# carry4985/ORB_SLAM2_MAP

Measured on AMD Instinct MI355X. Metric: frames/sec ORB extract+match (640x480, 1000 feat), higher is better.
Workload: dtype u8; 1 GPU; C2: synthetic 640x480 RGB-D stream, 1000 features, 8 levels, extract + BF-Hamming match of consecutive frames; resident_frame_pool=1024, sequences=1, parallelism=1 sequence per GPU, schedule_name=best, extraction_parts=1

## Files before the change

### orb_slam2_map_amd/csrc/extractor.hip

```cpp
#include "common.h"

#include <atomic>
#include <chrono>
#include <thread>
#include <tuple>
#include <type_traits>
#include <utility>
#include "trig_base.h"
#include "pyramid_view.h"

#include <algorithm>
#include <cfloat>
#include <cmath>
#include <cstdlib>
#include <cstring>
#include <vector>

namespace orbgpu {

constexpr int EDGE = 19;
constexpr int BORDER0 = EDGE - 3;
constexpr int HALF_PATCH = 15;
constexpr int PATCH = 31;
constexpr float CELL_W = 30.f;
// ... 59 lines not shown

struct Src0 {
    const uint8_t *p;
    size_t frame_stride;
    uint32_t pitch;
    int direct;
};
constexpr int BLUR0_OX = EDGE + 1;

__device__ __forceinline__ uint32_t rowoff(int row, int pitch) { return __umul24((unsigned)row, (unsigned)pitch); }

constexpr int PYR_ROWS = 8;

__global__ __launch_bounds__(256) void k_border0(const uint8_t *__restrict__ src, size_t stride,
                                                 size_t frame_stride, uint8_t *__restrict__ pyr,
                                                 size_t frame_pyr, const LevelGeom *__restrict__ geom)
{
    const LevelGeom g = geom[0];
    const int ndw = g.pitch >> 2;
    int bx, f;
    xcd_frame_block(bx, f);
    const int item = bx * 256 + threadIdx.x;
    const int rg = item / ndw;
    const int x4 = (item - rg * ndw) * 4;
    if (rg * PYR_ROWS >= g.h + 2 * EDGE)
        return;
    const int sx0 = x4 - EDGE;
    const bool interior = sx0 >= 0 && sx0 + 7 < g.w;
#pragma unroll 4
    for (int rr = 0; rr < PYR_ROWS; rr++) {
        const int py = rg * PYR_ROWS + rr;
        if (py >= g.h + 2 * EDGE)
            break;
        const int sy = reflect101(py - EDGE, g.h);
        const uint8_t *s = src + (size_t)f * frame_stride + __umul24((unsigned)sy, (unsigned)stride);
        uint32_t v = 0;
        if (interior && ((reinterpret_cast<uintptr_t>(s) & 3) == 0)) {
            const uint32_t *s32 = reinterpret_cast<const uint32_t *>(s) + (sx0 >> 2);
            v = __builtin_amdgcn_alignbyte(s32[1], s32[0], sx0 & 3);
        } else {
#pragma unroll
            for (int k = 0; k < 4; k++) {
                int px = min(x4 + k, g.w + 2 * EDGE - 1);
                int sx = reflect101(px - EDGE, g.w);
                v |= (uint32_t)s[sx] << (8 * k);
            }
        }
        *reinterpret_cast<uint32_t *>(pyr + (size_t)f * frame_pyr + g.plane_off + rowoff(py, g.pitch) + x4) = v;
    }
}

constexpr int BORDER_ROWS = 4;

struct BorderCol {
    uint32_t d;
    uint32_t sel;
};

__global__ __launch_bounds__(256) void k_border0_fast(const uint8_t *__restrict__ src, size_t stride, size_t frame_stride,
                                                      uint8_t *__restrict__ pyr, size_t frame_pyr,
                                                      const LevelGeom *__restrict__ geom,
                                                      const BorderCol *__restrict__ cols)
{
    const LevelGeom g = geom[0];
    const int n16 = g.pitch >> 4;
    int bx, f;
    xcd_frame_block(bx, f);
    const int item = bx * 256 + threadIdx.x;
    const int rg = item / n16;
    const int c16 = item - rg * n16;
    if (rg * BORDER_ROWS >= g.h + 2 * EDGE)
        return;
    const uint4 t01 = reinterpret_cast<const uint4 *>(cols)[c16 * 2], t23 = reinterpret_cast<const uint4 *>(cols)[c16 * 2 + 1];
    const uint8_t *sf = src + (size_t)f * frame_stride;
    uint8_t *dst = pyr + (size_t)f * frame_pyr + g.plane_off + c16 * 16;
    const bool interior = c16 >= 2 && c16 * 16 - EDGE + 15 < g.w - 1 && c16 * 4 - 5 + 4 < (g.w >> 2);
    struct __attribute__((packed, aligned(4))) Win {
        uint32_t d[5];
    };
    if (interior) {
        Win wn[BORDER_ROWS];
#pragma unroll
        for (int rr = 0; rr < BORDER_ROWS; rr++) {
            const int py = min(rg * BORDER_ROWS + rr, g.h + 2 * EDGE - 1);
            wn[rr] = *reinterpret_cast<const Win *>(sf + __umul24((unsigned)reflect101(py - EDGE, g.h), (unsigned)stride) +
                                                    (c16 * 16 - 20));
        }
#pragma unroll
        for (int rr = 0; rr < BORDER_ROWS; rr++) {
            const int py = rg * BORDER_ROWS + rr;
            if (py >= g.h + 2 * EDGE)
                break;
            uint4 v;
            v.x = __builtin_amdgcn_alignbyte(wn[rr].d[1], wn[rr].d[0], 1);
            v.y = __builtin_amdgcn_alignbyte(wn[rr].d[2], wn[rr].d[1], 1);
            v.z = __builtin_amdgcn_alignbyte(wn[rr].d[3], wn[rr].d[2], 1);
            v.w = __builtin_amdgcn_alignbyte(wn[rr].d[4], wn[rr].d[3], 1);
            *reinterpret_cast<uint4 *>(dst + rowoff(py, g.pitch)) = v;
        }
        return;
    }
#pragma unroll
    for (int rr = 0; rr < BORDER_ROWS; rr++) {
        const int py = rg * BORDER_ROWS + rr;
        if (py >= g.h + 2 * EDGE)
            break;
        const uint32_t *s32 = reinterpret_cast<const uint32_t *>(sf + __umul24((unsigned)reflect101(py - EDGE, g.h), (unsigned)stride));
        uint4 v;
        v.x = __builtin_amdgcn_perm(s32[t01.x + 1], s32[t01.x], t01.y);
        v.y = __builtin_amdgcn_perm(s32[t01.z + 1], s32[t01.z], t01.w);
        v.z = __builtin_amdgcn_perm(s32[t23.x + 1], s32[t23.x], t23.y);
        v.w = __builtin_amdgcn_perm(s32[t23.z + 1], s32[t23.z], t23.w);
        *reinterpret_cast<uint4 *>(dst + rowoff(py, g.pitch)) = v;
    }
}

__global__ __launch_bounds__(256) void k_resize_level(uint8_t *__restrict__ pyr, size_t frame_pyr,
                                                      const LevelGeom *__restrict__ geom, int level,
                                                      const XTab *__restrict__ xtab,
                                                      const YTab *__restrict__ ytab)
{
    const LevelGeom g = geom[level];
    const LevelGeom gs = geom[level - 1];
    const int x4 = (blockIdx.x * 256 + threadIdx.x) * 4;
    const int py = blockIdx.y;
    const int f = blockIdx.z;
    if (x4 >= g.pitch)
        return;
    const int dy = reflect101(py - EDGE, g.h);
    const YTab yt = ytab[g.ytab_off + dy];
    const uint8_t *base = pyr + (size_t)f * frame_pyr + gs.plane_off + rowoff(EDGE, gs.pitch) + EDGE;
    const uint8_t *S0 = base + rowoff(yt.sy0, gs.pitch);
    const uint8_t *S1 = base + rowoff(yt.sy1, gs.pitch);
    uint32_t v = 0;
#pragma unroll
    for (int k = 0; k < 4; k++) {
        int px = min(x4 + k, g.w + 2 * EDGE - 1);
        int dx = reflect101(px - EDGE, g.w);
        const XTab xt = xtab[g.xtab_off + dx];
        int t0 = S0[xt.sx] * xt.a0 + S0[xt.sx1] * xt.a1;
        int t1 = S1[xt.sx] * xt.a0 + S1[xt.sx1] * xt.a1;
        int o = ((((int)yt.b0 * (t0 >> 4)) >> 16) + (((int)yt.b1 * (t1 >> 4)) >> 16) + 2) >> 2;
        v |= (uint32_t)(o & 0xFF) << (8 * k);
    }
    *reinterpret_cast<uint32_t *>(pyr + (size_t)f * frame_pyr + g.plane_off + rowoff(py, g.pitch) + x4) = v;
}

struct ResizeStrip {
    uint32_t base_q;
};

typedef unsigned short us2 __attribute__((ext_vector_type(2)));

template <bool REUSE, bool DIRECT>
__global__ __launch_bounds__(256) void k_resize_fast(uint8_t *__restrict__ pyr, size_t frame_pyr,
                                                     const LevelGeom *__restrict__ geom, int level,
                                                     const ResizeStrip *__restrict__ strips,
                                                     const uint4 *__restrict__ sels, const uint4 *__restrict__ wts,
                                                     const YRow *__restrict__ yrows, int strip_off, int rows, Src0 s0)
{
    const LevelGeom g = geom[level];
    const LevelGeom gs = geom[level - 1];
    const int ndw = g.pitch >> 2;
    int bx, f;
    xcd_frame_block(bx, f);
    const int item = bx * 256 + threadIdx.x;
    const int rg = item / ndw;
    const int sdw = item - rg * ndw;
    if (rg * rows >= g.h + 2 * EDGE)
        return;
    const uint32_t bq = strips[strip_off + sdw].base_q;
    const uint32_t sh = (bq >> 16) & 3u;
    const uint4 sel = sels[strip_off + sdw], wt = wts[strip_off + sdw];
    const uint32_t selv[4] = {sel.x, sel.y, sel.z, sel.w}, wv[4] = {wt.x, wt.y, wt.z, wt.w};
    uint8_t *fb = pyr + (size_t)f * frame_pyr;
    const uint8_t *sb = DIRECT ? s0.p + (size_t)f * s0.frame_stride : fb;
    const int spitch = DIRECT ? (int)s0.pitch : gs.pitch;
    const uint32_t base = (DIRECT ? 0u : (uint32_t)gs.plane_off + (uint32_t)EDGE * (uint32_t)gs.pitch) + (bq & 0xFFFFu);
    const bool edge = DIRECT && ((bq >> 18) & 1u) != 0u;
    const uint32_t dst = (uint32_t)g.plane_off + (uint32_t)sdw * 4u;
    YRow yts[PYR_ROWS];
#pragma unroll
    for (int rr = 0; rr < PYR_ROWS; rr++)
        yts[rr] = yrows[g.yrow_off + min(rg * rows + rr, g.h + 2 * EDGE - 1)];
    int kept_row = -1, kept[4] = {0, 0, 0, 0};
#pragma unroll
    for (int rr = 0; rr < PYR_ROWS; rr++) {
        const int py = rg * rows + rr;
        if (rr >= rows || py >= g.h + 2 * EDGE)
            break;
        const YRow yt = yts[rr];
        const uint32_t *S1 = reinterpret_cast<const uint32_t *>(sb + (base + rowoff(yt.sy1, spitch)));
        uint32_t c0 = S1[0], c1 = S1[1];
        const uint32_t c2 = S1[2];
        if (DIRECT) {
            c0 = edge ? c1 : c0;
            c1 = edge ? c2 : c1;
        }
        int t0[4];
        if (!REUSE || yt.sy0 != kept_row) {
            const uint32_t *S0 = reinterpret_cast<const uint32_t *>(sb + (base + rowoff(yt.sy0, spitch)));
            uint32_t a0 = S0[0], a1 = S0[1];
            const uint32_t a2 = S0[2];
            if (DIRECT) {
                a0 = edge ? a1 : a0;
                a1 = edge ? a2 : a1;
            }
            const uint32_t lo = __builtin_amdgcn_alignbyte(a1, a0, sh), hi = __builtin_amdgcn_alignbyte(a2, a1, sh);
#pragma unroll
            for (int k = 0; k < 4; k++) {
                const uint32_t p0 = __builtin_amdgcn_perm(hi, lo, selv[k]);
                t0[k] = (int)__builtin_amdgcn_udot2(__builtin_bit_cast(us2, p0), __builtin_bit_cast(us2, wv[k]), 0u, false);
            }
        } else {
#pragma unroll
            for (int k = 0; k < 4; k++)
                t0[k] = kept[k];
        }
        uint32_t v = 0;
        const uint32_t lo1 = __builtin_amdgcn_alignbyte(c1, c0, sh), hi1 = __builtin_amdgcn_alignbyte(c2, c1, sh);
#pragma unroll
        for (int k = 0; k < 4; k++) {
            const uint32_t p1 = __builtin_amdgcn_perm(hi1, lo1, selv[k]);
            const int t1 = (int)__builtin_amdgcn_udot2(__builtin_bit_cast(us2, p1), __builtin_bit_cast(us2, wv[k]), 0u, false);
            const int o = ((__mul24(yt.b0, t0[k] >> 4) >> 16) + (__mul24(yt.b1, t1 >> 4) >> 16) + 2) >> 2;
            v |= (uint32_t)o << (8 * k);
            kept[k] = t1;
        }
        kept_row = yt.sy1;
        *reinterpret_cast<uint32_t *>(fb + (dst + rowoff(py, g.pitch))) = v;
    }
}

constexpr int MAX_CELL = 66;

typedef short pk16 __attribute__((ext_vector_type(2)));
__device__ __forceinline__ pk16 as_pk(uint32_t u) { return __builtin_bit_cast(pk16, u); }
__device__ __forceinline__ uint32_t as_u32(pk16 v) { return __builtin_bit_cast(uint32_t, v); }
__device__ __forceinline__ pk16 pkmin(pk16 a, pk16 b) { return __builtin_elementwise_min(a, b); }
__device__ __forceinline__ pk16 pkmax(pk16 a, pk16 b) { return __builtin_elementwise_max(a, b); }

typedef _Float16 pkh __attribute__((ext_vector_type(2)));
__device__ __forceinline__ pkh as_h(pk16 v) { return __builtin_bit_cast(pkh, v); }
__device__ __forceinline__ pk16 h_as_pk(pkh v) { return __builtin_bit_cast(pk16, v); }
__device__ __forceinline__ pkh hmax3(pkh a, pkh b, pkh c)
{
    return __builtin_elementwise_maximum(__builtin_elementwise_maximum(a, b), c);
}
__device__ __forceinline__ pkh hmin3(pkh a, pkh b, pkh c)
{
    return __builtin_elementwise_minimum(__builtin_elementwise_minimum(a, b), c);
}

__device__ __forceinline__ pk16 fast_score_pk(pk16 c, const pk16 p[16])
{
    pkh v[16], m2[8], m4[8], t[8];
#pragma unroll
    for (int k = 0; k < 16; k++)
        v[k] = as_h(p[k]);
#pragma unroll
    for (int i = 0; i < 8; i++)
        m2[i] = __builtin_elementwise_maximum(v[2 * i + 1], v[(2 * i + 2) & 15]);
#pragma unroll
    for (int i = 0; i < 8; i++)
        m4[i] = __builtin_elementwise_maximum(m2[i], m2[(i + 1) & 7]);
#pragma unroll
    for (int i = 0; i < 8; i++)
        t[i] = hmax3(m4[i], m4[(i + 2) & 7], __builtin_elementwise_minimum(v[2 * i], v[(2 * i + 9) & 15]));
    const pkh A = __builtin_elementwise_minimum(hmin3(hmin3(t[0], t[1], t[2]), hmin3(t[3], t[4], t[5]), t[6]), t[7]);
#pragma unroll
    for (int i = 0; i < 8; i++)
        m2[i] = __builtin_elementwise_minimum(v[2 * i + 1], v[(2 * i + 2) & 15]);
#pragma unroll
    for (int i = 0; i < 8; i++)
        m4[i] = __builtin_elementwise_minimum(m2[i], m2[(i + 1) & 7]);
#pragma unroll
    for (int i = 0; i < 8; i++)
        t[i] = hmin3(m4[i], m4[(i + 2) & 7], __builtin_elementwise_maximum(v[2 * i], v[(2 * i + 9) & 15]));
    const pkh B = __builtin_elementwise_maximum(hmax3(hmax3(t[0], t[1], t[2]), hmax3(t[3], t[4], t[5]), t[6]), t[7]);
    typedef unsigned short pku16 __attribute__((ext_vector_type(2)));
    const pku16 cu = __builtin_bit_cast(pku16, c);
    const pku16 dk = __builtin_elementwise_sub_sat(cu, __builtin_bit_cast(pku16, A));
    const pku16 br = __builtin_elementwise_sub_sat(__builtin_bit_cast(pku16, B), cu);
    return __builtin_bit_cast(pk16, __builtin_elementwise_max(dk, br));
}

#define ORBGPU_SEL_EVEN(o) ((uint32_t)(o) | 0x0c00u | ((uint32_t)((o) + 2) << 16) | 0x0c000000u)
#define ORBGPU_SEL_ODD(o) ((uint32_t)((o) + 1) | 0x0c00u | ((uint32_t)((o) + 3) << 16) | 0x0c000000u)

struct Row3 {
    uint32_t d[3];
};

struct RowU {
    uint32_t f[8];
};
__device__ __forceinline__ void unpack_row(const Row3 &R, RowU &U)
{
#pragma unroll
    for (int o = 1; o <= 8; o++) {
        const int q = o >> 2;
        U.f[o - 1] = __builtin_amdgcn_perm(R.d[q < 2 ? q + 1 : 2], R.d[q], ORBGPU_SEL_EVEN(o & 3));
    }
}
template <int DX, int ODD> __device__ __forceinline__ pk16 ring_half(const RowU &R)
{
    return as_pk(R.f[4 + DX + ODD - 1]);
}

template <int ODD>
__device__ __forceinline__ pk16 fast_score_half(const RowU &r0, const RowU &r1, const RowU &r2, const RowU &r3,
                                                const RowU &r4, const RowU &r5, const RowU &r6)
{
    pk16 p[16];
    const pk16 c = ring_half<0, ODD>(r3);
    p[0] = ring_half<0, ODD>(r6);
    p[1] = ring_half<1, ODD>(r6);
    p[2] = ring_half<2, ODD>(r5);
    p[3] = ring_half<3, ODD>(r4);
    p[4] = ring_half<3, ODD>(r3);
    p[5] = ring_half<3, ODD>(r2);
    p[6] = ring_half<2, ODD>(r1);
    p[7] = ring_half<1, ODD>(r0);
    p[8] = ring_half<0, ODD>(r0);
    p[9] = ring_half<-1, ODD>(r0);
    p[10] = ring_half<-2, ODD>(r1);
    p[11] = ring_half<-3, ODD>(r2);
    p[12] = ring_half<-3, ODD>(r3);
    p[13] = ring_half<-3, ODD>(r4);
    p[14] = ring_half<-2, ODD>(r5);
    p[15] = ring_half<-1, ODD>(r6);
    return fast_score_pk(c, p);
}

template <int ODD>
__device__ __forceinline__ uint32_t fast_maybe_half(const RowU &r0, const RowU &r3, const RowU &r6, pkh tpk)
{
    const pkh c = as_h(ring_half<0, ODD>(r3));
    const pkh p0 = as_h(ring_half<0, ODD>(r6)), p4 = as_h(ring_half<3, ODD>(r3));
    const pkh p8 = as_h(ring_half<0, ODD>(r0)), p12 = as_h(ring_half<-3, ODD>(r3));
    const pkh bm = hmax3(__builtin_elementwise_minimum(p0, p4), __builtin_elementwise_minimum(p4, p8),
                         __builtin_elementwise_maximum(__builtin_elementwise_minimum(p8, p12), __builtin_elementwise_minimum(p12, p0)));
    const pkh dm = hmin3(__builtin_elementwise_maximum(p0, p4), __builtin_elementwise_maximum(p4, p8),
                         __builtin_elementwise_minimum(__builtin_elementwise_maximum(p8, p12), __builtin_elementwise_maximum(p12, p0)));
    const pk16 ci = h_as_pk(c), ti = h_as_pk(tpk);
    const uint32_t eb = as_u32((ci + ti) - h_as_pk(bm));
    const uint32_t ed = as_u32(h_as_pk(dm) - (ci - ti));
    return (eb | ed) & 0x80008000u;
}

struct StripGeom {
    int first[ORBGPU_MAX_LEVELS + 1];
    int nsx[ORBGPU_MAX_LEVELS];
    int nlevels;
};


constexpr int FD_OWN = 62;
constexpr int FD_QCAP = 512;
constexpr int FD_CELLS = 32;
constexpr int FD_EARLY_HOLD = 3;

struct DetectGeom {
    int first[ORBGPU_MAX_LEVELS + 1];
    int nsx[ORBGPU_MAX_LEVELS];
    int ncols[ORBGPU_MAX_LEVELS];
    int ctab_off[ORBGPU_MAX_LEVELS];
    int xfirst[ORBGPU_MAX_LEVELS];
    int nlevels;
};

struct ColumnInfo {
    uint32_t cellj;
    uint32_t flags;
};

struct DetectLane {
    int xrel, yrel;
    int cell_base;
    uint32_t cellj;
};

// ... 1953 lines not shown
    hipGraph_t graph = nullptr;
    hipGraphNode_t last = nullptr;
    hipError_t err = hipSuccess;

    Launcher() = default;
    explicit Launcher(hipStream_t s) : st(s) {}

    template <typename... P, typename... A> void launch(void (*kern)(P...), dim3 grid, dim3 block, size_t lds, A &&...a)
    {
        static_assert(sizeof...(P) == sizeof...(A), "kernel argument count");
        if (!graph) {
            hipLaunchKernelGGL(kern, grid, block, lds, st, static_cast<P>(a)...);
            return;
        }
        std::tuple<std::remove_cv_t<P>...> vals(static_cast<P>(a)...);
        void *ptrs[sizeof...(P) + 1];
        fill(ptrs, vals, std::index_sequence_for<P...>{});
        hipKernelNodeParams kp = {};
        kp.func = reinterpret_cast<void *>(kern);
        kp.gridDim = grid;
        kp.blockDim = block;
        kp.sharedMemBytes = (unsigned)lds;
        kp.kernelParams = ptrs;
        kp.extra = nullptr;
        add([&](hipGraphNode_t *n, const hipGraphNode_t *dep, size_t ndep) { return hipGraphAddKernelNode(n, graph, dep, ndep, &kp); });
    }
    int memset32(void *dst, size_t bytes)
    {
        if (!graph) {
            ORBGPU_HIP_TRY(hipMemsetAsync(dst, 0, bytes, st));
            return ORBGPU_OK;
        }
        hipMemsetParams mp = {};
        mp.dst = dst;
        mp.elementSize = 4;
        mp.width = bytes / 4;
        mp.height = 1;
        mp.pitch = bytes;
        mp.value = 0;
        add([&](hipGraphNode_t *n, const hipGraphNode_t *dep, size_t ndep) { return hipGraphAddMemsetNode(n, graph, dep, ndep, &mp); });
        return ORBGPU_OK;
    }

private:
    template <typename T, size_t... I> static void fill(void **ptrs, T &vals, std::index_sequence<I...>)
    {
        ((ptrs[I] = const_cast<void *>(static_cast<const void *>(&std::get<I>(vals)))), ...);
    }
    template <typename F> void add(F f)
    {
        hipGraphNode_t n = nullptr;
        const hipError_t e = f(&n, last ? &last : nullptr, last ? 1 : 0);
        if (e != hipSuccess && err == hipSuccess)
            err = e;
        if (e == hipSuccess)
            last = n;
    }
};

static int materialize_level0(orbgpu_extractor *e, const Src0 &s0, int batch, Launcher &L)
{
    const LevelGeom &g = e->geom[0];
    const LevelGeom *dg = e->d_geom.as<LevelGeom>();
    uint8_t *pyr = e->d_pyr.as<uint8_t>();
    const size_t stride = s0.pitch;
    if (e->border_fast && stride % 4 == 0 && s0.frame_stride % 4 == 0 && (reinterpret_cast<uintptr_t>(s0.p) & 3) == 0) {
        dim3 gridf(((g.pitch / 16) * ((g.h + 2 * EDGE + BORDER_ROWS - 1) / BORDER_ROWS) + 255) / 256, batch);
        L.launch(k_border0_fast, gridf, dim3(256), 0, s0.p, stride, s0.frame_stride, pyr, e->frame_pyr, dg,
                           e->d_bcol.as<BorderCol>());
    } else {
        dim3 grid(((g.pitch / 4) * ((g.h + 2 * EDGE + PYR_ROWS - 1) / PYR_ROWS) + 255) / 256, batch);
        L.launch(k_border0, grid, dim3(256), 0, s0.p, stride, s0.frame_stride, pyr, e->frame_pyr, dg);
    }
    if (!L.graph)
        ORBGPU_HIP_TRY(hipGetLastError());
    return ORBGPU_OK;
}

static void launch_blur(orbgpu_extractor *e, const Src0 &s0, int batch, Launcher &L, int which = 0)
{
    const int nl = e->nlevels;
    const LevelGeom *dg = e->d_geom.as<LevelGeom>();
    uint8_t *pyr = e->d_pyr.as<uint8_t>(), *blur = e->d_blur.as<uint8_t>();
    int strip0 = 0;
    if (s0.direct) {
        const LevelGeom &g = e->geom[0];
        const int nstrips = (g.w / 8) * ((g.h + BLUR_ROWS - 1) / BLUR_ROWS);
        if (which != 2)
            L.launch(k_blur0_direct, dim3((nstrips + 255) / 256, batch), dim3(256), 0, s0, blur, e->frame_pyr, dg);
        strip0 = e->blur_geom.first[1];
    }
    if (which == 1)
        return;
    if (e->blur_geom.first[nl] > strip0)
        L.launch(k_blur, dim3((e->blur_geom.first[nl] - strip0 + 255) / 256, batch), dim3(256), 0, pyr, blur,
                           e->frame_pyr, dg, e->blur_geom, strip0);
}

static int launch_pipeline(orbgpu_extractor *e, const uint8_t *d_gray, int batch, int w, int h, size_t stride,
                           size_t frame_stride, orbgpu_keypoint *d_kps, uint8_t *d_desc, int cap, int *d_n_out,
                           Launcher &L)
{
    hipStream_t st = L.st;
    const int nl = e->nlevels;
    const LevelGeom *dg = e->d_geom.as<LevelGeom>();
    uint8_t *pyr = e->d_pyr.as<uint8_t>();
    uint8_t *blur = e->d_blur.as<uint8_t>();
    int rc = e->d_aux.reserve(sizeof(KpAux) * (size_t)cap * batch);
    if (rc != ORBGPU_OK)
        return rc;
    const bool rec = L.graph != nullptr;
    const bool prof = !rec && e->profiling && e->prof_calls < orbgpu_extractor::PROF_SLOTS;
    if (prof && e->ev.empty()) {
        e->ev.resize((size_t)orbgpu_extractor::PROF_SLOTS * 2 * ST_COUNT, nullptr);
        for (auto &x : e->ev)
            ORBGPU_HIP_TRY(hipEventCreate(&x));
    }
    hipEvent_t *evs = prof ? &e->ev[(size_t)e->prof_calls * 2 * ST_COUNT] : nullptr;
#define BEGIN(stage, s) if (prof && (stage) == 0) ORBGPU_HIP_TRY(hipEventRecord(evs[0], s))
#define END(stage, s)                                                          \
    {                                                                          \
        if (prof)                                                              \
            ORBGPU_HIP_TRY(hipEventRecord(evs[1 + (stage)], s));               \
        if (!rec && e->stage_signal[stage])                                    \
            ORBGPU_HIP_TRY(hipEventRecord(e->stage_signal[stage], s));         \
        if (!rec && e->pipe_signal[stage])                                     \
            ORBGPU_HIP_TRY(hipEventRecord(e->pipe_signal[stage], s));          \
    }
    const bool aligned4 = stride % 4 == 0 && frame_stride % 4 == 0 && (reinterpret_cast<uintptr_t>(d_gray) & 3) == 0;
    const bool direct = e->direct0_ok && !e->no_direct0 && aligned4 && batch >= e->direct0_min_batch;
    const Src0 s0{d_gray, frame_stride, (uint32_t)stride, direct ? 1 : 0};
    e->last_src = s0;
    e->level0_materialized = !direct;
    BEGIN(ST_PYRAMID, st);
    const bool side_blur = e->concurrent_blur && !rec;
    Launcher Ls(e->side);
    const bool early_blur0 = side_blur && direct && !e->no_early_blur0;
    if (early_blur0) {
        ORBGPU_HIP_TRY(hipEventRecord(e->ev_fork0, st));
        ORBGPU_HIP_TRY(hipStreamWaitEvent(e->side, e->ev_fork0, 0));
        if (prof)
            ORBGPU_HIP_TRY(hipEventRecord(evs[ST_COUNT + 1], e->side));
        launch_blur(e, s0, batch, Ls, 1);
    }
    {
        if (!direct) {
            int rcb = materialize_level0(e, s0, batch, L);
            if (rcb != ORBGPU_OK)
                return rcb;
        }
        for (int l = 1; l < nl; l++) {
            const LevelGeom &gl = e->geom[l];
            dim3 gr((gl.pitch / 4 + 255) / 256, gl.h + 2 * EDGE, batch);
            const int ndw_l = (gl.pitch / 4) * (gl.h + 2 * EDGE);
            const int rows = ndw_l >= 32768 ? PYR_ROWS : ndw_l >= 16384 ? PYR_ROWS / 2 : PYR_ROWS / 4;
            dim3 grf(((gl.pitch / 4) * ((gl.h + 2 * EDGE + rows - 1) / rows) + 255) / 256, batch);
            if (gl.rs_fast) {
                const bool dir1 = direct && l == 1;
                auto kern = dir1 ? (rows == PYR_ROWS ? k_resize_fast<true, true> : k_resize_fast<false, true>)
                                 : (rows == PYR_ROWS ? k_resize_fast<true, false> : k_resize_fast<false, false>);
                L.launch(kern, grf, dim3(256), 0, pyr, e->frame_pyr, dg, l, e->d_rstrip.as<ResizeStrip>(),
                                   e->d_rsel.as<uint4>(), e->d_rwt.as<uint4>(), e->d_yrow.as<YRow>(),
                                   dir1 ? e->rs_off_direct : gl.rs_off, rows, s0);
            }
            else
                L.launch(k_resize_level, gr, dim3(256), 0, pyr, e->frame_pyr, dg, l,
                                   e->d_xtab.as<XTab>(), e->d_ytab.as<YTab>());
        }
    }
    END(ST_PYRAMID, st);
    BEGIN(ST_BLUR, st);
    if (side_blur) {
        ORBGPU_HIP_TRY(hipEventRecord(e->ev_fork, st));
        ORBGPU_HIP_TRY(hipStreamWaitEvent(e->side, e->ev_fork, 0));
        if (prof && !early_blur0)
            ORBGPU_HIP_TRY(hipEventRecord(evs[ST_COUNT + 1], e->side));
        launch_blur(e, s0, batch, Ls, early_blur0 ? 2 : 0);
        if (prof)
            ORBGPU_HIP_TRY(hipEventRecord(evs[ST_COUNT + 2], e->side));
        ORBGPU_HIP_TRY(hipEventRecord(e->ev_join, e->side));
    } else
        launch_blur(e, s0, batch, L);
    END(ST_BLUR, st);
    BEGIN(ST_FAST, st);
    if (e->counters_dirty) {
        int rcm = L.memset32(e->d_cellcnt.p, e->d_cellcnt.bytes & ~(size_t)3);
        if (rcm == ORBGPU_OK)
            rcm = L.memset32(e->d_qtaux.p, e->d_qtaux.bytes & ~(size_t)3);
        if (rcm != ORBGPU_OK)
            return rcm;
    }
    e->counters_dirty = true;
    {
        const int t_ini = std::max(e->prm.ini_th_fast, 1), t_min = std::max(e->prm.min_th_fast, 1);
        const DetectGeom &dgeo = direct ? e->det_geom_direct : e->det_geom;
        const int nwaves = (dgeo.first[nl] + FD_OWN - 1) / FD_OWN;
        L.launch(e->fast_early_out ? k_fast_detect<true> : k_fast_detect<false>, dim3((nwaves + 3) / 4, batch), dim3(256), 0, pyr, e->frame_pyr, dg,
                           dgeo, e->d_ctab.as<ColumnInfo>(), e->d_cells.as<CellDesc>(), (int)e->cells.size(),
                           e->d_slots.as<uint32_t>(), e->frame_slots, e->d_cellcnt.as<int>(), std::min(t_ini, t_min),
                           t_ini, e->fast_queue_cap, s0);
    }
    END(ST_FAST, st);
    BEGIN(ST_QUADTREE, st);
    if (batch >= QT_BATCH_MIN || e->force_batch_quadtree)
        L.launch(k_quadtree<false>, dim3(batch, nl), dim3(QT_THREADS_BATCH), e->qt_lds, dg,
                           e->d_cells.as<CellDesc>(), (int)e->cells.size(), e->d_slots.as<uint32_t>(), e->frame_slots,
                           e->d_cellcnt.as<int>(), e->d_dkey.as<uint32_t>(), e->d_dnode.as<uint16_t>(),
                           e->d_sel.as<uint32_t>(), e->sel_cap_total, e->d_nsel.as<int>(), e->d_ncand.as<int>(), nl,
                           e->ncap, std::max(e->prm.ini_th_fast, 1), 0, qt_dbg(), (int *)nullptr);
    else {
        if (e->qt_prefilter)
            L.launch(k_qt_prefilter, dim3(std::min((e->max_slots_level + QT_PRE_KEYS - 1) / QT_PRE_KEYS, QT_PRE_GRID), nl, batch), dim3(256), 0, dg, (int)e->cells.size(), e->d_slots.as<uint32_t>(), e->frame_slots, e->d_cellcnt.as<int>(),
                               e->d_dkey.as<uint32_t>(), e->d_qtaux.as<int>(), std::max(e->prm.ini_th_fast, 1));
        L.launch(k_quadtree<true>, dim3(batch, nl), dim3(w * h >= QT_LARGE_PIXELS ? QT_THREADS : QT_THREADS_SMALL), e->qt_lds + (size_t)e->qt_kcap * 6, dg,
                           e->d_cells.as<CellDesc>(), (int)e->cells.size(), e->d_slots.as<uint32_t>(), e->frame_slots,
                           e->d_cellcnt.as<int>(), e->d_dkey.as<uint32_t>(), e->d_dnode.as<uint16_t>(),
                           e->d_sel.as<uint32_t>(), e->sel_cap_total, e->d_nsel.as<int>(), e->d_ncand.as<int>(), nl,
                           e->ncap, std::max(e->prm.ini_th_fast, 1), e->qt_kcap, qt_dbg(),
                           e->qt_prefilter ? e->d_qtaux.as<int>() : (int *)nullptr);
    }
    if (!rec)
        ORBGPU_HIP_TRY(hipGetLastError());
    e->counters_dirty = false;
    END(ST_QUADTREE, st);
    BEGIN(ST_ORIENT, st);
    const int or_iters = batch >= OR_BATCH_MIN ? OR_ITERS : 1;
    L.launch(k_orient, dim3((e->sel_cap_total + 8 * or_iters - 1) / (8 * or_iters), batch), dim3(256), 0, pyr, e->frame_pyr, dg, nl,
                       e->d_sel.as<uint32_t>(), e->sel_cap_total, e->d_nsel.as<int>(),
                       reinterpret_cast<const uint32_t *>(e->d_pattern.as<uint8_t>() + 1024), d_kps,
                       e->d_aux.as<KpAux>(), cap, d_n_out, or_iters, s0);
    L.launch(k_trig, dim3((std::min(cap, e->max_kp) + 255) / 256, batch), dim3(256), 0,
                       e->d_aux.as<KpAux>(), d_n_out, cap, e->trig);
    END(ST_ORIENT, st);
    BEGIN(ST_DESCRIBE, st);
    if (side_blur)
        ORBGPU_HIP_TRY(hipStreamWaitEvent(st, e->ev_join, 0));
    L.launch(k_describe, dim3((std::min(cap, e->max_kp) + 7) / 8, batch), dim3(256), 0, blur,
                       e->frame_pyr, dg, e->d_aux.as<KpAux>(), d_n_out, cap, e->d_pattern.as<int8_t>(), d_desc);
    END(ST_DESCRIBE, st);
#undef BEGIN
#undef END
    if (!rec)
        ORBGPU_HIP_TRY(hipGetLastError());
    else if (L.err != hipSuccess) {
        set_error("recording the extraction graph: %s", hipGetErrorString(L.err));
        return ORBGPU_EHIP;
    }
    if (prof)
        e->prof_calls++;
    e->last_batch = batch;
    e->last_cap = cap;
    (void)w;
    (void)h;
    return ORBGPU_OK;
}

}

namespace orbgpu {

int extractor_pyramid_view(const orbgpu_extractor *e, PyramidView *v)
{
    ORBGPU_REQUIRE(e && v, "null argument");
    memset(v, 0, sizeof(*v));
    v->device_id = e->prm.device_id;
    v->nlevels = e->nlevels;
    v->scale_factor = e->prm.scale_factor;
    v->last_batch = (int)e->geom.size() == e->nlevels ? e->last_batch : 0;
    for (int l = 0; l < e->nlevels; l++) {
        v->scale[l] = e->scale[l];
        v->inv_scale[l] = e->inv_scale[l];
        if (v->last_batch > 0) {
            const LevelGeom &g = e->geom[l];
            v->w[l] = g.w;
            v->h[l] = g.h;
            v->pitch[l] = g.pitch;
            v->plane_off[l] = g.plane_off;
        }
    }
    v->pyr = e->d_pyr.as<uint8_t>();
    v->frame_pyr = e->frame_pyr;
    v->border = EDGE;
    v->direct = v->last_batch > 0 && e->last_src.direct ? 1 : 0;
    v->l0 = v->direct ? e->last_src.p : nullptr;
    v->l0_frame_stride = v->direct ? e->last_src.frame_stride : 0;
    v->l0_pitch = v->direct ? e->last_src.pitch : 0;
    v->scratch = &e->d_stereo;
    return ORBGPU_OK;
}

}

extern "C" {

int orbgpu_extractor_create(const orbgpu_extractor_params *p, orbgpu_extractor **out)
{
    std::lock_guard<std::mutex> lifecycle(orbgpu::lifecycle_mutex());
    ORBGPU_REQUIRE(p && out, "null argument");
    ORBGPU_REQUIRE(p->nlevels >= 1 && p->nlevels <= ORBGPU_MAX_LEVELS, "nlevels must be in [1,%d]", ORBGPU_MAX_LEVELS);
    ORBGPU_REQUIRE(p->nfeatures >= 1, "nfeatures must be positive");
    ORBGPU_REQUIRE(p->scale_factor > 1.0f, "scale_factor must be > 1");
    ORBGPU_REQUIRE(p->ini_th_fast >= 0 && p->ini_th_fast <= 255 && p->min_th_fast >= 0 && p->min_th_fast <= 255,
                   "FAST thresholds must be in [0,255]");
    int rc = select_device(p->device_id);
    if (rc != ORBGPU_OK)
        return rc;
    orbgpu_extractor *e = new (std::nothrow) orbgpu_extractor();
    if (!e) {
        set_error("out of host memory");
        return ORBGPU_ENOMEM;
    }
    e->prm = *p;
    if (e->prm.max_batch < 1)
        e->prm.max_batch = 1;
    e->force_batch_quadtree = getenv("ORBGPU_DEBUG_QT_BATCH") != nullptr;
    e->qt_no_prefilter = getenv("ORBGPU_DEBUG_QT_NOPRE") != nullptr;
// ... 625 lines not shown
```

Before: 290,700 frames/s.

## Batch all resize source-row loads up front and fix rows per thread

The fast resize kernel now issues all source-row window loads for its PYR_ROWS output rows before doing any arithmetic, with a compiler fence so the loads stay grouped and their latency overlaps. Row reuse is decided statically from the y-table (own_up), replacing the runtime kept_row check. The host-side heuristic that used fewer rows per thread on small levels is removed, so every level uses PYR_ROWS rows per thread. This raises memory-level parallelism per thread but costs more registers and fewer threads on the small pyramid levels.

```diff
diff --git a/orb_slam2_map_amd/csrc/extractor.hip b/orb_slam2_map_amd/csrc/extractor.hip
--- a/orb_slam2_map_amd/csrc/extractor.hip
+++ b/orb_slam2_map_amd/csrc/extractor.hip
@@ -235,12 +235,12 @@
 
 typedef unsigned short us2 __attribute__((ext_vector_type(2)));
 
-template <bool REUSE, bool DIRECT>
+template <bool DIRECT>
 __global__ __launch_bounds__(256) void k_resize_fast(uint8_t *__restrict__ pyr, size_t frame_pyr,
                                                      const LevelGeom *__restrict__ geom, int level,
                                                      const ResizeStrip *__restrict__ strips,
                                                      const uint4 *__restrict__ sels, const uint4 *__restrict__ wts,
-                                                     const YRow *__restrict__ yrows, int strip_off, int rows, Src0 s0)
+                                                     const YRow *__restrict__ yrows, int strip_off, Src0 s0)
 {
     const LevelGeom g = geom[level];
     const LevelGeom gs = geom[level - 1];
@@ -250,7 +250,8 @@
     const int item = bx * 256 + threadIdx.x;
     const int rg = item / ndw;
     const int sdw = item - rg * ndw;
-    if (rg * rows >= g.h + 2 * EDGE)
+    const int nprow = g.h + 2 * EDGE;
+    if (rg * PYR_ROWS >= nprow)
         return;
     const uint32_t bq = strips[strip_off + sdw].base_q;
     const uint32_t sh = (bq >> 16) & 3u;
@@ -265,26 +266,44 @@
     YRow yts[PYR_ROWS];
 #pragma unroll
     for (int rr = 0; rr < PYR_ROWS; rr++)
-        yts[rr] = yrows[g.yrow_off + min(rg * rows + rr, g.h + 2 * EDGE - 1)];
-    int kept_row = -1, kept[4] = {0, 0, 0, 0};
+        yts[rr] = yrows[g.yrow_off + min(rg * PYR_ROWS + rr, nprow - 1)];
+    struct Win3 {
+        uint32_t d0, d1, d2;
+    };
+    Win3 lw[PYR_ROWS], uw[PYR_ROWS];
+    bool own_up[PYR_ROWS];
 #pragma unroll
     for (int rr = 0; rr < PYR_ROWS; rr++) {
-        const int py = rg * rows + rr;
-        if (rr >= rows || py >= g.h + 2 * EDGE)
+        const uint32_t *S1 = reinterpret_cast<const uint32_t *>(sb + (base + rowoff(yts[rr].sy1, spitch)));
+        lw[rr] = Win3{S1[0], S1[1], S1[2]};
+    }
+#pragma unroll
+    for (int rr = 0; rr < PYR_ROWS; rr++) {
+        own_up[rr] = rr == 0 || yts[rr].sy0 != yts[rr - 1].sy1;
+        uw[rr] = Win3{0u, 0u, 0u};
+        if (own_up[rr]) {
+            const uint32_t *S0 = reinterpret_cast<const uint32_t *>(sb + (base + rowoff(yts[rr].sy0, spitch)));
+            uw[rr] = Win3{S0[0], S0[1], S0[2]};
+        }
+    }
+    __atomic_signal_fence(__ATOMIC_SEQ_CST);
+    int kept[4] = {0, 0, 0, 0};
+#pragma unroll
+    for (int rr = 0; rr < PYR_ROWS; rr++) {
+        const int py = rg * PYR_ROWS + rr;
+        if (py >= nprow)
             break;
         const YRow yt = yts[rr];
-        const uint32_t *S1 = reinterpret_cast<const uint32_t *>(sb + (base + rowoff(yt.sy1, spitch)));
-        uint32_t c0 = S1[0], c1 = S1[1];
-        const uint32_t c2 = S1[2];
+        uint32_t c0 = lw[rr].d0, c1 = lw[rr].d1;
+        const uint32_t c2 = lw[rr].d2;
         if (DIRECT) {
             c0 = edge ? c1 : c0;
             c1 = edge ? c2 : c1;
         }
         int t0[4];
-        if (!REUSE || yt.sy0 != kept_row) {
-            const uint32_t *S0 = reinterpret_cast<const uint32_t *>(sb + (base + rowoff(yt.sy0, spitch)));
-            uint32_t a0 = S0[0], a1 = S0[1];
-            const uint32_t a2 = S0[2];
+        if (own_up[rr]) {
+            uint32_t a0 = uw[rr].d0, a1 = uw[rr].d1;
+            const uint32_t a2 = uw[rr].d2;
             if (DIRECT) {
                 a0 = edge ? a1 : a0;
                 a1 = edge ? a2 : a1;
@@ -310,7 +329,6 @@
             v |= (uint32_t)o << (8 * k);
             kept[k] = t1;
         }
-        kept_row = yt.sy1;
         *reinterpret_cast<uint32_t *>(fb + (dst + rowoff(py, g.pitch))) = v;
     }
 }
@@ -2570,16 +2588,12 @@
         for (int l = 1; l < nl; l++) {
             const LevelGeom &gl = e->geom[l];
             dim3 gr((gl.pitch / 4 + 255) / 256, gl.h + 2 * EDGE, batch);
-            const int ndw_l = (gl.pitch / 4) * (gl.h + 2 * EDGE);
-            const int rows = ndw_l >= 32768 ? PYR_ROWS : ndw_l >= 16384 ? PYR_ROWS / 2 : PYR_ROWS / 4;
-            dim3 grf(((gl.pitch / 4) * ((gl.h + 2 * EDGE + rows - 1) / rows) + 255) / 256, batch);
+            dim3 grf(((gl.pitch / 4) * ((gl.h + 2 * EDGE + PYR_ROWS - 1) / PYR_ROWS) + 255) / 256, batch);
             if (gl.rs_fast) {
                 const bool dir1 = direct && l == 1;
-                auto kern = dir1 ? (rows == PYR_ROWS ? k_resize_fast<true, true> : k_resize_fast<false, true>)
-                                 : (rows == PYR_ROWS ? k_resize_fast<true, false> : k_resize_fast<false, false>);
-                L.launch(kern, grf, dim3(256), 0, pyr, e->frame_pyr, dg, l, e->d_rstrip.as<ResizeStrip>(),
-                                   e->d_rsel.as<uint4>(), e->d_rwt.as<uint4>(), e->d_yrow.as<YRow>(),
-                                   dir1 ? e->rs_off_direct : gl.rs_off, rows, s0);
+                L.launch(dir1 ? k_resize_fast<true> : k_resize_fast<false>, grf, dim3(256), 0, pyr, e->frame_pyr, dg, l,
+                                   e->d_rstrip.as<ResizeStrip>(), e->d_rsel.as<uint4>(), e->d_rwt.as<uint4>(), e->d_yrow.as<YRow>(),
+                                   dir1 ? e->rs_off_direct : gl.rs_off, s0);
             }
             else
                 L.launch(k_resize_level, gr, dim3(256), 0, pyr, e->frame_pyr, dg, l,
```

Result: no change. 293,100 frames/s, median of 4 (+0.8%).
